# the-lay/voltools

Hardware: AMD Instinct MI355X
Metric: Mvoxels/s, 512^3 f32 filt_bspline StaticVolume transform (resident source, device output) (higher is better)
Workload: dtype f32; 1 GPU; 512^3 float32 filt_bspline, StaticVolume resident in HBM, rotate((0,i,0)) rzxz sweep, output= device buffer; lds_bytes=34816, kernel=8, resident_bytes=1660944384, angles=i

## Files before the change

include/voltools_hip.h:

```cpp
#ifndef VOLTOOLS_HIP_H
#define VOLTOOLS_HIP_H

#include <stddef.h>
#include <stdint.h>

#ifdef __cplusplus
extern "C" {
#endif

enum vt_interp {
    VT_LINEAR = 0,
    VT_BSPLINE = 1,
    VT_BSPLINE_SIMPLE = 2,
    VT_FILT_BSPLINE = 3,
    VT_FILT_BSPLINE_SIMPLE = 4
};

enum vt_flags {
    VT_OUT_DEVICE = 1,
    VT_KEEP_OUTSIDE = 2,
    VT_FORCE_DIRECT = 4,
    VT_FORCE_TILED = 8,
    VT_NO_ZSEP = 16,
    VT_NO_MARCH = 32,
    VT_NO_ZPAIR = 64,
    VT_NO_PACKED = 128,
    VT_FORCE_PACKED = 256,
    VT_FORCE_XSWAP = 512,
    VT_NO_RSWAP = 1024,
    VT_ONESHOT_EDGE_SCIPY = 4096,
    VT_NO_QUAD = 2048,
    VT_NO_BLOCK = 8192,
    VT_NO_ZFIR = 16384,
    VT_NO_REORIENT = 32768,
    VT_NO_ROWS = 65536,
    VT_NO_PLANSHARE = 131072
};

enum vt_create_flags {
    VT_SRC_DEVICE = 1,
    VT_SLAB_LO_INTERIOR = 2,
    VT_SLAB_HI_INTERIOR = 4,
    VT_EDGE_SCIPY = 16,
    VT_SRC_DEFERRED = 8
};

enum vt_error {
    VT_OK = 0,
    VT_EINVAL = 10001,
    VT_ENODEV = 10002,
    VT_ENOMEM = 10003,
    VT_EUNSUPPORTED = 10004
};

typedef struct vt_volume vt_volume_t;

typedef struct vt_volume_info {
    int32_t device;
    int32_t interp;
    int32_t depth, height, width;
    int32_t out_depth, out_height, out_width;
    int32_t last_kernel;
    int32_t last_tile[3];
    int32_t last_lds_dims[3];
    int32_t last_lds_bytes;
    int32_t last_grid;
    float   prefilter_ms;
    uint64_t resident_bytes;
    float   copies_ms;
    int32_t copies_built;
    int32_t copies_evicted;
    uint64_t max_resident_bytes;
} vt_volume_info_t;

int vt_device_count(int* count);
int vt_device_name(int dev, char* buf, int buflen);
int vt_device_props(int dev, int* cu_count, int* lds_bytes_per_block, uint64_t* hbm_bytes);
int vt_device_synchronize(int dev);

int vt_malloc(int dev, size_t bytes, void** dptr);
int vt_free(int dev, void* dptr);
int vt_memset_zero(int dev, void* dptr, size_t bytes);
int vt_memcpy_h2d(int dev, void* dptr, const void* hptr, size_t bytes);
int vt_memcpy_d2h(int dev, void* hptr, const void* dptr, size_t bytes);
int vt_memcpy_d2d(int dev, void* dst, const void* src, size_t bytes);
int vt_host_register(int dev, void* ptr, size_t bytes);
int vt_host_unregister(int dev, void* ptr);
int vt_device_trim(int dev);

// ... 73 lines not shown
```

voltools_amd/_native.py:

```python
import ctypes
import os
from typing import Optional, Tuple

import numpy as np

_HERE = os.path.dirname(os.path.abspath(__file__))
LIB_PATH = os.environ.get('VT_LIB') or os.path.join(_HERE, 'lib', 'libvoltools_hip.so')

INTERP_CODES = {'linear': 0, 'bspline': 1, 'bspline_simple': 2, 'filt_bspline': 3, 'filt_bspline_simple': 4}

OUT_DEVICE, KEEP_OUTSIDE, FORCE_DIRECT, FORCE_TILED, NO_ZSEP, NO_MARCH, NO_ZPAIR, NO_PACKED, FORCE_PACKED, FORCE_XSWAP, NO_RSWAP, NO_QUAD, ONESHOT_EDGE_SCIPY, NO_BLOCK, NO_ZFIR, NO_REORIENT, NO_ROWS, NO_PLANSHARE = 1, 2, 4, 8, 16, 32, 64, 128, 256, 512, 1024, 2048, 4096, 8192, 16384, 32768, 65536, 131072
SRC_DEVICE, SLAB_LO_INTERIOR, SLAB_HI_INTERIOR, SRC_DEFERRED, EDGE_SCIPY = 1, 2, 4, 8, 16

SYMBOLS = [
    'vt_device_count', 'vt_device_name', 'vt_device_props', 'vt_device_synchronize',
    'vt_malloc', 'vt_free', 'vt_memset_zero', 'vt_memcpy_h2d', 'vt_memcpy_d2h', 'vt_memcpy_d2d',
    'vt_host_register', 'vt_host_unregister', 'vt_device_trim',
    'vt_volume_create', 'vt_volume_create_slab', 'vt_volume_upload_planes', 'vt_volume_finalize', 'vt_volume_destroy', 'vt_volume_info', 'vt_volume_stream',
    'vt_volume_sync', 'vt_volume_set_output_shape', 'vt_volume_affine', 'vt_volume_affine_f64',
    'vt_volume_project', 'vt_volume_project_f64', 'vt_volume_affine_batch',
    'vt_timer_start', 'vt_timer_stop', 'vt_prefilter_inplace', 'vt_affine_oneshot',
    'vt_last_error', 'vt_version', 'vt_has_legacy_kernels', 'vt_volume_release_copies', 'vt_volume_set_max_resident',
    'vt_volume_extract', 'vt_volume_extract_f64', 'vt_volume_project_batch', 'vt_volume_project_batch_f64',
    'vt_volume_extract_sum', 'vt_volume_extract_sum_f64', 'vt_volume_extract_dot', 'vt_volume_extract_dot_f64',
    'vt_volume_extract_dot_multi', 'vt_volume_extract_dot_multi_f64',
]


class VolumeInfo(ctypes.Structure):
    _fields_ = [('device', ctypes.c_int32), ('interp', ctypes.c_int32),
                ('depth', ctypes.c_int32), ('height', ctypes.c_int32), ('width', ctypes.c_int32),
                ('out_depth', ctypes.c_int32), ('out_height', ctypes.c_int32), ('out_width', ctypes.c_int32),
                ('last_kernel', ctypes.c_int32), ('last_tile', ctypes.c_int32 * 3),
                ('last_lds_dims', ctypes.c_int32 * 3), ('last_lds_bytes', ctypes.c_int32),
                ('last_grid', ctypes.c_int32), ('prefilter_ms', ctypes.c_float),
                ('resident_bytes', ctypes.c_uint64), ('copies_ms', ctypes.c_float), ('copies_built', ctypes.c_int32),
                ('copies_evicted', ctypes.c_int32), ('max_resident_bytes', ctypes.c_uint64)]


_lib = None


def _preload_hip_runtime():
    import importlib.util
    import sys
    if os.environ.get('VT_HIP_RUNTIME', '') == 'system' or 'torch' in sys.modules:
        return
    try:
        spec = importlib.util.find_spec('torch')
    except (ImportError, ValueError):
        spec = None
    if spec is None or not spec.submodule_search_locations:
        return
    cand = os.path.join(list(spec.submodule_search_locations)[0], 'lib', 'libamdhip64.so')
    if os.path.exists(cand):
        try:
            ctypes.CDLL(cand, mode=ctypes.RTLD_GLOBAL)
        except OSError:
            pass


def load():
    global _lib
    if _lib is not None:
# ... 278 lines not shown
```

voltools_amd/csrc/vt_kernels_quad.hip:

```cpp
#include "vt_internal.h"
#include <cstdio>
#include <cstdlib>
#include <mutex>
#include <unordered_map>
#include "vt_device.h"
#include "vt_march_common.h"

#include <type_traits>

namespace vt {

typedef float v4f __attribute__((ext_vector_type(4)));

constexpr int kQuadMaxIt = 5;

template <int NT> constexpr int quad_plan_granules() { return (kTabInts + NT * kQuadMaxIt / 4 + 2) / 3; }
constexpr int quad_plan_vote_off(int granules) { return kTabBytes + ((12 * granules + 15) & ~15); }
constexpr int quad_plan_lds_bytes(int granules, int nt) { return quad_plan_vote_off(granules) + 4 * (nt / 64); }

__global__ __launch_bounds__(256) void relayout_zquad(const float* __restrict__ src, float* __restrict__ dst,
                                                       int D, int H, int W, int P, int Pq)
{
    const int x = blockIdx.x * 256 + threadIdx.x;
    const int y = blockIdx.y;
// ... 150 lines not shown
                    const float x0 = fmaf(fx, a01 - a00, a00);
                    const float x1 = fmaf(fx, a11 - a10, a10);
                    pl[c] = fmaf(fy, x1 - x0, x0);
                }
                val = fmaf(p.fz, pl[1] - pl[0], pl[0]);
            } else if constexpr (KIND == 4) {
                const int z = d + p.zoff;
                float accy = 0.f;
#pragma unroll
                for (int bb = 0; bb < 4; ++bb) {
                    const int y = gy0 - 1 + bb;
                    float accx = wx[0] * fetch(z, y, gx0 - 1);
                    accx = fmaf(wx[1], fetch(z, y, gx0), accx);
                    accx = fmaf(wx[2], fetch(z, y, gx0 + 1), accx);
                    accx = fmaf(wx[3], fetch(z, y, gx0 + 2), accx);
                    accy = fmaf(wy[bb], accx, accy);
                }
                val = accy;
            } else {
#pragma unroll
                for (int c = 0; c < 4; ++c) {
                    const int z = d + p.zoff - 1 + c;
                    float accy = 0.f;
#pragma unroll
                    for (int bb = 0; bb < 4; ++bb) {
                        const int y = gy0 - 1 + bb;
                        float accx = wx[0] * fetch(z, y, gx0 - 1);
                        accx = fmaf(wx[1], fetch(z, y, gx0), accx);
                        accx = fmaf(wx[2], fetch(z, y, gx0 + 1), accx);
                        accx = fmaf(wx[3], fetch(z, y, gx0 + 2), accx);
                        accy = fmaf(wy[bb], accx, accy);
                    }
                    val = (c == 0) ? wz[0] * accy : fmaf(wz[c], accy, val);
                }
            }
            out[oo + (int64_t)d * p.ostride] = val;
        } else if (!keep) out[oo + (int64_t)d * p.ostride] = 0.0f;
    }
}

__device__ __forceinline__ int quad_lane_to_pos(int lane)
{
    const int blk = (lane >> 2) & 7;
    const int sh = (int)((0x30051663u >> (4 * blk)) & 15u) - 3;
    return lane + 4 * sh;
}
__device__ __forceinline__ int quad_pos_to_lane(int pos)
{
    const int blk = (pos >> 2) & 7;
    const int sh = (int)((0x31006653u >> (4 * blk)) & 15u) - 3;
    return pos + 4 * sh;
}

template <int KIND, int TH, int TW, int NT>
__global__ __launch_bounds__(NT, (KIND == 4 && TH * TW == 2 * NT) ? 4 : 1) void affine_march4(const float* __restrict__ srcq, float* __restrict__ out, const AffineParams p)
{
    static_assert(NT % TW == 0 && TH % (NT / TW) == 0 && NT % 64 == 0 && 64 % TW == 0, "tile/thread mapping");
    static_assert(NT == 256 || NT == 512, "quad_tile_plan_granules");
    static_assert(quad_plan_granules<NT>() <= NT && 3 * quad_plan_granules<NT>() <= kTabInts + kVrowCap / 4, "one plan granule per thread");
    constexpr bool CUBIC = KIND == 1 || KIND == 2 || KIND == 4;
    constexpr bool ZID = KIND == 3 || KIND == 4;
    constexpr int HALO = CUBIC ? 1 : 0;
    constexpr int ZH = ZID ? 0 : HALO;
    constexpr int NR = 2 + 2 * HALO;
    constexpr int NC = 2 * ZH + 1;
    constexpr int ZNEW = ZID ? 0 : 1;
    constexpr int RP = NT / TW;
    constexpr int NPIX = TH / RP;
    constexpr int NSTORE = 4 * NPIX;
    extern __shared__ __attribute__((aligned(16))) float lds[];

    const int tid = threadIdx.x;
#ifdef VT_EXPERIMENTS
    if ((p.flags & (1 << 27)) && (p.flags & (1 << 26))) return;
    long long stamp[5];
    stamp[0] = clock64();
#endif
    int tw_i, th_i, chunk;
    if (p.flags & (1 << 29)) {
        chunk = (p.flags & (1 << 20)) ? (int)(gridDim.y - 1 - blockIdx.y) : (int)blockIdx.y;
        unsigned u = (unsigned)xcd_contiguous(blockIdx.x, gridDim.x);
        if (p.flags & (1 << 30)) u = gridDim.x - 1 - u;
        if (p.flags & (1 << 24)) {
            tw_i = (int)__umulhi(u, p.nTh_magic);
            th_i = (int)u - tw_i * p.nTh;
        } else {
            th_i = (int)__umulhi(u, p.nTw_magic);
            tw_i = (int)u - th_i * p.nTw;
        }
    } else {
        int t = xcd_contiguous(blockIdx.x, gridDim.x);
        if (p.flags & (1 << 20)) t = (int)gridDim.x - 1 - t;
        march_tile(p, t, th_i, tw_i, chunk);
    }
    const int h0 = th_i * TH, w0 = tw_i * TW;
    constexpr int PG = quad_plan_granules<NT>();
    const bool share = KIND == 4 && p.tplan != nullptr;
    int4 pgran = {0, 0, 0, 0};
    int4* const plan_g = share ? reinterpret_cast<int4*>(p.tplan) + (int64_t)(th_i * p.nTw + tw_i) * PG : nullptr;
    if (share && tid < PG) {
        const __amdgpu_buffer_rsrc_t prsrc = __builtin_amdgcn_make_buffer_rsrc(plan_g, 0, PG * 16, 0x00020000);
        pgran = __builtin_bit_cast(int4, __builtin_amdgcn_raw_buffer_load_b128(prsrc, 16 * tid, 0, 16));
    }
    const int d_begin = chunk ? chunk * p.dch + p.dshift : 0;
    const int d_end = min((chunk + 1) * p.dch + p.dshift, p.oD);

    double base[3], lo[3], hi[3];
    bool any_valid = true, all_valid = true;
#pragma unroll
    for (int r = 1; r < 3; ++r) {
        base[r] = fma(p.m[4 * r + 1], (double)h0, fma(p.m[4 * r + 2], (double)w0, p.m[4 * r + 3]));
        lo[r] = base[r] + p.neg[r];
        hi[r] = base[r] + p.pos[r];
        any_valid = any_valid && (hi[r] >= p.vlo[r] - kTileMargin) && (lo[r] < p.vhi[r] + kTileMargin);
        all_valid = all_valid && (lo[r] >= p.vlo[r] + kTileMargin) && (hi[r] < p.vhi[r] - kTileMargin);
    }
    const double z_lo = (double)d_begin + p.m[3], z_hi = (double)(d_end - 1) + p.m[3];
    any_valid = any_valid && (z_hi >= p.vlo[0] - kTileMargin) && (z_lo < p.vhi[0] + kTileMargin);
    all_valid = all_valid && (z_lo >= p.vlo[0] + kTileMargin) && (z_hi < p.vhi[0] - kTileMargin);
    const bool keep = (p.flags & VT_KEEP_OUTSIDE) != 0;
    const int64_t ostride = p.ostride, orow = p.orow;
    const bool lane_perm = (p.flags & (1 << 23)) != 0;
    const int lane_id = tid & 63;
    const int pos = lane_perm ? quad_lane_to_pos(lane_id) : lane_id;
    const int kw = pos % TW;
    const int jh0 = (tid >> 6) * (64 / TW) + pos / TW;
    const int lane_left = lane_perm ? quad_pos_to_lane((pos + 63) & 63) : ((lane_id + 63) & 63);
    const int lane_right = lane_perm ? quad_pos_to_lane((pos + 1) & 63) : ((lane_id + 1) & 63);

    if (!any_valid) {
        if (!keep) {
#pragma unroll
            for (int px = 0; px < NPIX; ++px) {
                const int h = h0 + jh0 + px * RP, w = w0 + kw;
                if (h < p.oH && w < p.oW) {
                    float* optr = out + (int64_t)d_begin * ostride + (int64_t)h * orow + w;
                    for (int d = d_begin; d < d_end; ++d, optr += ostride) *optr = 0.0f;
                }
            }
        }
        return;
    }

    int o1, o2;
    {
        const int f1 = (int)floor(lo[1]), f2 = (int)floor(lo[2]);
        int g1 = f1, g2 = f2;
        asm volatile("" : "+v"(g1), "+v"(g2));
        o1 = __builtin_amdgcn_readfirstlane(g1);
        o2 = __builtin_amdgcn_readfirstlane(g2);
        o1 -= HALO;
        o2 -= HALO;
    }

    int iy[NPIX], ix[NPIX];
    float fy[NPIX], fx[NPIX];
    float wy[NPIX][4], wx[NPIX][4];
    bool in_yx[NPIX], pix_ok[NPIX];
    int ob[NPIX];
    const double by = base[1] - (double)o1, bx = base[2] - (double)o2;
#pragma unroll
    for (int px = 0; px < NPIX; ++px) {
        const int j = jh0 + px * RP;
        const double sy = fma(p.m[5], (double)j, fma(p.m[6], (double)kw, by));
        const double sx = fma(p.m[9], (double)j, fma(p.m[10], (double)kw, bx));
        const double fyd = floor(sy), fxd = floor(sx);
        fy[px] = (float)(sy - fyd);
        fx[px] = (float)(sx - fxd);
        iy[px] = (int)fyd;
        ix[px] = (int)fxd;
        if constexpr (KIND == 4) {
            if (p.flags & (1 << 18)) { cubic_weights<true>(fy[px], wy[px]); cubic_weights<true>(fx[px], wx[px]); }
            else { cubic_weights<false>(fy[px], wy[px]); cubic_weights<false>(fx[px], wx[px]); }
        } else if constexpr (CUBIC) { cubic_weights<KIND == 2>(fy[px], wy[px]); cubic_weights<KIND == 2>(fx[px], wx[px]); }
        else {
#pragma unroll
            for (int k = 0; k < 4; ++k) { wy[px][k] = 0.f; wx[px][k] = 0.f; }
        }
        in_yx[px] = all_valid || (canonical_inside_axis(p, 1, 0, h0 + j, w0 + kw) && canonical_inside_axis(p, 2, 0, h0 + j, w0 + kw));
        pix_ok[px] = (h0 + j < p.oH) && (w0 + kw < p.oW);
        ob[px] = (int)(((int64_t)j * orow + kw) * 4);
    }

#ifdef VT_EXPERIMENTS
    stamp[1] = clock64();
#endif
    int voff[kQuadMaxIt];
    int q[NPIX][NR];
    int nvec;
    {
        int* tab = reinterpret_cast<int*>(lds);
#ifdef VT_QUAD_ANALYTIC_SPANS
        build_span_table<TH, TW, HALO, 1>(tab, p, p.Ly, by, bx, tid);
#else
        if (tid < 2 * kRowsMax) tab[tid] = (tid < kRowsMax) ? 0x7fffffff : (int)0x80000000;
        int* const img = reinterpret_cast<int*>(reinterpret_cast<char*>(lds) + kTabBytes);
        int* const vote = reinterpret_cast<int*>(reinterpret_cast<char*>(lds) + quad_plan_vote_off(PG));
        if (share) {
            if (tid < PG) { img[3 * tid] = pgran.x; img[3 * tid + 1] = pgran.y; img[3 * tid + 2] = pgran.z; }
            const bool wave_ok = __all(tid >= PG || (unsigned)pgran.w == p.tplan_epoch);
            if ((tid & 63) == 0) vote[tid >> 6] = wave_ok ? 1 : 0;
        }
        __syncthreads();
        bool hit = false;
        if (share) {
            int all = 1;
#pragma unroll
            for (int w = 0; w < NT / 64; ++w) all &= vote[w];
            hit = __builtin_amdgcn_readfirstlane(all) != 0;
        }
        if (hit) {
            tab = img;
#ifdef VT_EXPERIMENTS
            stamp[2] = stamp[3] = clock64();
#endif
        } else {
            unsigned char* vrow = reinterpret_cast<unsigned char*>(tab + kTabInts);
#pragma unroll
            for (int px = 0; px < NPIX; ++px) {
                const int iy_l = __shfl(iy[px], lane_left), iy_r = __shfl(iy[px], lane_right);
                const bool edge = (kw == 0) || (kw == TW - 1) || (iy_l != iy[px]) || (iy_r != iy[px]);
                if (edge) {
#pragma unroll
                    for (int r = 0; r < NR; ++r) {
                        const int row = min(max(iy[px] - HALO + r, 0), kRowsMax - 1);
                        atomicMin(&tab[row], ix[px] - HALO);
                        atomicMax(&tab[kRowsMax + row], ix[px] + HALO + 1);
                    }
                }
            }
            __syncthreads();
#ifdef VT_EXPERIMENTS
            stamp[2] = clock64();
#endif
            if (tid < kRowsMax) {
                const int lane = tid;
                const int mn = tab[lane], mx = tab[kRowsMax + lane];
                const bool used = mn <= mx;
                const int x0 = used ? mn : 0;
                const int nv = used ? (mx - mn + 1) : 0;
                int first, pad = 0, total;
                {
                    const int incl = wave_scan_add(nv);
                    first = incl - nv;
                    total = __builtin_amdgcn_readlane(incl, 63);
                }
                if (p.row_s >= 0) {
                    const int S = p.row_s;
                    const int c_r = (x0 + lane * S) & 15;
                    const int end_res = (nv > 0) ? ((c_r + nv) & 15) : 0;
                    const int last_used = wave_scan_max((nv > 0) ? lane : -1);
                    const int prev_row = wave_shift_up1(last_used, -1);
                    int prev_end = __shfl(end_res, max(prev_row, 0));
                    if (lane == 0 || prev_row < 0) prev_end = 0;
                    const int gap = (nv > 0) ? ((c_r - prev_end) & 15) : 0;
                    const int inc2 = wave_scan_add(gap + nv);
// ... 9 lines not shown
                int v = first;
                for (; v < last && (v & 3); ++v) vrow[v] = (unsigned char)lane;
                const unsigned lane4 = (unsigned)lane * 0x01010101u;
                for (; v + 4 <= last; v += 4) *reinterpret_cast<unsigned*>(vrow + v) = lane4;
                for (; v < last; ++v) vrow[v] = (unsigned char)lane;
            }
            __syncthreads();
#ifdef VT_EXPERIMENTS
            stamp[3] = clock64();
#endif
            if (share && tid < PG) {
                const int nvb = min(tab[2 * kRowsMax], NT * kQuadMaxIt);
                int w[3];
#pragma unroll
                for (int j = 0; j < 3; ++j) {
                    const int k = 3 * tid + j;
                    const int b = 4 * (k - kTabInts);
                    int val = 0;
                    if (k <= 2 * kRowsMax) val = tab[k];
                    else if (k >= kTabInts && b < nvb) val = tab[k] & ((b + 4 <= nvb) ? -1 : (int)((1u << (8 * (nvb - b))) - 1u));
                    w[j] = val;
                }
                plan_g[tid] = make_int4(w[0], w[1], w[2], (int)p.tplan_epoch);
            }
        }
#endif
        const unsigned char* vrow = reinterpret_cast<const unsigned char*>(tab + kTabInts);
        nvec = tab[2 * kRowsMax];
#pragma unroll
        for (int it = 0; it < kQuadMaxIt; ++it) {
            const int v = tid + NT * it;
            const int y = (v < nvec && v < kVrowCap) ? vrow[v] : 255;
            const int yy = (y == 255) ? 0 : y;
            const int cx = v - tab[kRowsMax + yy];
            const int gy = o1 + yy, gx = o2 + tab[yy] + cx;
            const bool ok = (y != 255) && (unsigned)gy < (unsigned)p.sH && (unsigned)gx < (unsigned)p.sW;
            voff[it] = ok ? (gy * p.sPq + 4 * gx) * 4 : p.zero_off_q;
        }
#pragma unroll
        for (int px = 0; px < NPIX; ++px) {
#pragma unroll
            for (int r = 0; r < NR; ++r) {
                const int row = min(max(iy[px] - HALO + r, 0), kRowsMax - 1);
                q[px][r] = 16 * (tab[kRowsMax + row] + (ix[px] - HALO - tab[row]));
            }
        }
        __syncthreads();
    }
#pragma unroll
    for (int it = 0; it < kQuadMaxIt; ++it) voff[it] -= p.zero_off_q;
    const int nvec64 = (nvec + 63) & ~63;
    const int slot_bytes = p.slot_floats * 4;

    if (nvec64 * 16 > slot_bytes || nvec64 > NT * kQuadMaxIt) {
#pragma unroll
        for (int px = 0; px < NPIX; ++px)
            if (pix_ok[px])
                quad_gather_column<KIND>(srcq, out, p, (int64_t)(h0 + jh0 + px * RP) * orow + (w0 + kw), d_begin, d_end, in_yx[px],
                                         o1 + iy[px], o2 + ix[px], fy[px], fx[px]);
        return;
    }

    const int wave_first = __builtin_amdgcn_readfirstlane(tid & ~63);
    const int quad_bytes = p.sH * p.sPq * 4;
    const int nquads_res = (p.sD + 3) >> 2;
    const int plane_first = d_begin + p.zoff - ZH, plane_last = d_end - 1 + p.zoff + ZH + ZNEW;
    const int Q0 = floordiv4(plane_first), QN = floordiv4(plane_last);
    const int Q_base = max(0, min(Q0, nquads_res - 1));
    __amdgpu_buffer_rsrc_t rsrc = __builtin_amdgcn_make_buffer_rsrc(
        const_cast<char*>(reinterpret_cast<const char*>(srcq) + (int64_t)Q_base * quad_bytes), 0, 0x7fffffff, 0x00020000);
    __amdgpu_buffer_rsrc_t orsrc = __builtin_amdgcn_make_buffer_rsrc(
        reinterpret_cast<char*>(out + ((int64_t)d_begin * ostride + (int64_t)h0 * orow + w0)), 0, 0x7fffffff, 0x00020000);
    const int oplane_bytes = (int)(ostride * 4);
    const float fz = p.fz;
    float wz[4] = {0.f, 0.f, 0.f, 0.f};
    if constexpr (CUBIC && !ZID) cubic_weights<KIND == 2>(fz, wz);
    const int tap_new = p.zoff + ZH + ZNEW;
    const int Qf0 = floordiv4(d_begin + tap_new + 3), Qf1 = floordiv4(d_end - 4 + tap_new);
    const bool nt_stores = (p.flags & (1 << 28)) != 0;
    const bool tile_fast = all_valid && (h0 + TH <= p.oH) && (w0 + TW <= p.oW);
    char* const lds_c = reinterpret_cast<char*>(lds);
#ifdef VT_EXPERIMENTS
    const bool no_stores = (p.flags & (1 << 21)) != 0, no_loads = (p.flags & (1 << 22)) != 0, no_lds = (p.flags & (1 << 26)) != 0;
#else
    constexpr bool no_stores = false, no_loads = false, no_lds = false;
#endif
#ifdef VT_EXPERIMENTS
    if (p.flags & (1 << 27)) {
        if (nvec == 12345678) out[0] = (float)(voff[0] + q[0][0]);
        stamp[4] = clock64();
        if (tid == 0) {
            const int64_t b = (int64_t)blockIdx.x + (int64_t)gridDim.x * blockIdx.y;
            for (int k = 0; k < 4; ++k) out[b * 4 + k] = (float)(stamp[k + 1] - stamp[k]);
        }
        return;
    }
#endif

    auto run = [&](auto nit_c) {
        constexpr int NIT = decltype(nit_c)::value;
        const bool last_wave = wave_first + NT * (NIT - 1) < nvec64;
        auto issue_quad = [&](int Q, int slot_off) {
            if (no_loads) return;
            const bool quad_ok = (unsigned)Q < (unsigned)nquads_res;
            const int soff = quad_ok ? (Q - Q_base) * quad_bytes : 0;
            const int okmask = quad_ok ? -1 : 0;
            char* dst = lds_c + slot_off + 16 * wave_first;
#pragma unroll
            for (int it = 0; it < NIT; ++it) {
                const int off = p.zero_off_q + (voff[it] & okmask);
                if (it + 1 < NIT || last_wave)
                    __builtin_amdgcn_raw_ptr_buffer_load_lds(rsrc, (__attribute__((address_space(3))) void*)(dst + (16 * NT) * it), 16, off, soff, 0, 0);
            }
        };

        float carry[NPIX][NC];
#pragma unroll
        for (int px = 0; px < NPIX; ++px)
#pragma unroll
            for (int c = 0; c < NC; ++c) carry[px][c] = 0.f;

        auto partials = [&](int slot_off, v4f (&part)[NPIX]) {
            if (no_lds) {
#pragma unroll
                for (int px = 0; px < NPIX; ++px) asm volatile("" : "=v"(part[px]));
                return;
            }
            const char* sl = lds_c + slot_off;
#pragma unroll
            for (int px = 0; px < NPIX; ++px) {
                if constexpr (!CUBIC) {
                    const v4f a00 = *reinterpret_cast<const v4f*>(sl + q[px][0]);
                    const v4f a01 = *reinterpret_cast<const v4f*>(sl + q[px][0] + 16);
                    const v4f a10 = *reinterpret_cast<const v4f*>(sl + q[px][1]);
                    const v4f a11 = *reinterpret_cast<const v4f*>(sl + q[px][1] + 16);
                    const v4f x0 = (a01 - a00) * fx[px] + a00;
                    const v4f x1 = (a11 - a10) * fx[px] + a10;
                    part[px] = (x1 - x0) * fy[px] + x0;
                } else {
                    v4f accy = {0.f, 0.f, 0.f, 0.f};
#pragma unroll
                    for (int bb = 0; bb < 4; ++bb) {
                        const char* rowp = sl + q[px][bb];
                        const v4f t0 = *reinterpret_cast<const v4f*>(rowp);
                        const v4f t1 = *reinterpret_cast<const v4f*>(rowp + 16);
                        const v4f t2 = *reinterpret_cast<const v4f*>(rowp + 32);
                        const v4f t3 = *reinterpret_cast<const v4f*>(rowp + 48);
                        v4f accx = t0 * wx[px][0];
                        accx = t1 * wx[px][1] + accx;
                        accx = t2 * wx[px][2] + accx;
                        accx = t3 * wx[px][3] + accx;
                        accy = accx * wy[px][bb] + accy;
                    }
                    part[px] = accy;
                }
            }
        };
        auto zcombine = [&](int px, float pn) -> float {
            float val;
            if constexpr (ZID) {
                val = pn;
            } else if constexpr (!CUBIC) {
                val = fmaf(fz, pn - carry[px][0], carry[px][0]);
                carry[px][0] = pn;
            } else {
                float acc = wz[0] * carry[px][0];
                acc = fmaf(wz[1], carry[px][1], acc);
                acc = fmaf(wz[2], carry[px][2], acc);
                val = fmaf(wz[3], pn, acc);
                carry[px][0] = carry[px][1]; carry[px][1] = carry[px][2]; carry[px][2] = pn;
            }
            return val;
        };

        int slot_off = 0;
        issue_quad(Q0, 0);
        bool prev_full = false;
        for (int Q = Q0; Q <= QN; ++Q) {
            const bool full = tile_fast && Q >= Qf0 && Q <= Qf1;
            if (full && prev_full && !no_stores) asm volatile("s_waitcnt vmcnt(%0)" ::"n"(NSTORE) : "memory");
            else asm volatile("s_waitcnt vmcnt(0)" ::: "memory");
            __builtin_amdgcn_s_barrier();
            if (Q < QN) issue_quad(Q + 1, slot_off ^ slot_bytes);
            v4f part[NPIX];
            partials(slot_off, part);
            const int d_first = 4 * Q - tap_new;
            if (full) {
                int soff = (d_first - d_begin) * oplane_bytes;
                float val[4][NPIX];
#pragma unroll
                for (int i = 0; i < 4; ++i)
#pragma unroll
                    for (int px = 0; px < NPIX; ++px) val[i][px] = zcombine(px, part[px][i]);
                if (no_stores) {
#pragma unroll
                    for (int i = 0; i < 4; ++i)
#pragma unroll
                        for (int px = 0; px < NPIX; ++px) asm volatile("" ::"v"(val[i][px]));
                } else if (nt_stores) {
#pragma unroll
                    for (int i = 0; i < 4; ++i, soff += oplane_bytes)
#pragma unroll
                        for (int px = 0; px < NPIX; ++px)
                            __builtin_amdgcn_raw_buffer_store_b32(__builtin_bit_cast(unsigned, val[i][px]), orsrc, ob[px], soff, 2);
                } else {
#pragma unroll
                    for (int i = 0; i < 4; ++i, soff += oplane_bytes)
#pragma unroll
                        for (int px = 0; px < NPIX; ++px)
                            __builtin_amdgcn_raw_buffer_store_b32(__builtin_bit_cast(unsigned, val[i][px]), orsrc, ob[px], soff, 0);
                }
            } else {
#pragma unroll
                for (int i = 0; i < 4; ++i) {
                    const int d = d_first + i;
                    const bool d_ok = (d >= d_begin) && (d < d_end);
                    const double ez = (double)d + p.m[3];
                    const bool z_ok = (ez >= p.vlo[0]) && (ez < p.vhi[0]);
                    const int soff = (d - d_begin) * oplane_bytes;
#pragma unroll
                    for (int px = 0; px < NPIX; ++px) {
                        const float val = zcombine(px, part[px][i]);
                        if (d_ok && pix_ok[px]) {
                            if (in_yx[px] && z_ok) __builtin_amdgcn_raw_buffer_store_b32(__builtin_bit_cast(unsigned, val), orsrc, ob[px], soff, 0);
                            else if (!keep) __builtin_amdgcn_raw_buffer_store_b32(0u, orsrc, ob[px], soff, 0);
                        }
                    }
                }
            }
            prev_full = full;
            slot_off ^= slot_bytes;
        }
    };
    using std::integral_constant;
    switch (nvec64 / NT + ((nvec64 % NT) ? 1 : 0)) {
        case 1: run(integral_constant<int, 1>{}); break;
        case 2: run(integral_constant<int, 2>{}); break;
        case 3: run(integral_constant<int, 3>{}); break;
        case 4: run(integral_constant<int, 4>{}); break;
        default: run(integral_constant<int, 5>{}); break;
    }
}

typedef void (*quad_fn)(const float*, float*, const AffineParams);
struct QuadCfg { int th, tw, nt; };
static const QuadCfg kQuad[] = {
    {16, 32, 256},
    {8, 32, 256},
    {32, 32, 256},
    {16, 64, 256},
    {32, 32, 512},
    {16, 64, 512},
};
int quad_max_it() { return kQuadMaxIt; }
int quad_config_count() { return (int)(sizeof(kQuad) / sizeof(kQuad[0])); }
void quad_config(int idx, int* th, int* tw, int* nt) { *th = kQuad[idx].th; *tw = kQuad[idx].tw; *nt = kQuad[idx].nt; }
int quad_tile_plan_granules(int cfg) { return kQuad[cfg].nt == 512 ? quad_plan_granules<512>() : quad_plan_granules<256>(); }
int quad_tile_plan_lds(int cfg) { return quad_plan_lds_bytes(quad_tile_plan_granules(cfg), kQuad[cfg].nt); }

template <int TH, int TW, int NT>
static quad_fn pick_quad(int kind)
{
    switch (kind) {
        case 0: return affine_march4<0, TH, TW, NT>;
        case 1: return affine_march4<1, TH, TW, NT>;
        case 3: return affine_march4<3, TH, TW, NT>;
        case 4: return affine_march4<4, TH, TW, NT>;
        default: return affine_march4<2, TH, TW, NT>;
    }
}
static quad_fn quad_entry(int cfg, int kind)
{
    switch (cfg) {
        case 0: return pick_quad<16, 32, 256>(kind);
        case 1: return pick_quad<8, 32, 256>(kind);
        case 2: return pick_quad<32, 32, 256>(kind);
        case 3: return pick_quad<16, 64, 256>(kind);
        case 4: return pick_quad<32, 32, 512>(kind);
        default: return pick_quad<16, 64, 512>(kind);
    }
}

hipError_t init_quad_kernels()
{
    for (int cfg = 0; cfg < quad_config_count(); ++cfg)
        for (int kind = 0; kind < 5; ++kind) {
            hipError_t e = hipFuncSetAttribute(reinterpret_cast<const void*>(quad_entry(cfg, kind)),
                                               hipFuncAttributeMaxDynamicSharedMemorySize, 160 * 1024);
            if (e != hipSuccess) return e;
        }
    return hipSuccess;
}

int quad_blocks_per_cu(int cfg, int interp, int lds_bytes, bool zid)
// ... 34 lines not shown
```

voltools_amd/csrc/vt_plan.hip:

```cpp
#include "vt_host.h"
#include "vt_device.h"

#include <cmath>
#include <cstring>

namespace vt {
namespace {

struct PlanCtx {
    const vt_volume* v;
    const double* m;
    int flags;
    AffineParams* p;
    TilePlan* plan;
    bool cubic;
    bool zsep;
    int halo2;
};

#ifdef VT_LEGACY
int64_t round_aware_chunks(int64_t oD, int g, int64_t inplane, int64_t resident, int64_t n0, int extra, int min_dch, int64_t n_floor)
{
    if (resident <= 0 || inplane > resident || inplane * n0 >= 16 * resident) return n0;
    auto cost = [&](int64_t n) {
// ... 230 lines not shown
                p->row_s = S;
                nvec64 = padded64;
            }
        }
        const int slot_bytes = nvec64 * 16;
        const int64_t bytes = std::max<int64_t>(2LL * slot_bytes, march_table_bytes());
        if (bytes > v->lds_limit) continue;
        c.plan->kind = 8; c.plan->cfg = cfg; c.plan->td = 4; c.plan->th = th; c.plan->tw = tw;
        c.plan->lds_bytes = (int)bytes;
        p->Lz = 2; p->Ly = std::min(L[1], march_rows_max()); p->Lx = npos; p->Lx_used = npos;
        p->slot_floats = slot_bytes / 4;
        return true;
    }
    return false;
}

bool plan_quad(PlanCtx& c)
{
    const vt_volume* v = c.v;
    AffineParams* p = c.p;
    TilePlan* plan = c.plan;
    if (!c.zsep || (c.flags & (VT_NO_MARCH | VT_NO_QUAD | VT_NO_ZPAIR))) return false;
    if (v->H > 65535 || (v->D + 3) / 4 > 65535) return false;
    const bool zfir = c.cubic && (float)(c.m[3] - std::floor(c.m[3])) == 0.0f && v->tune.quad_zfir != 0 && !(c.flags & VT_NO_ZFIR);
    const int halo = (c.cubic && !zfir) ? 1 : 0;
    const int Wq = (v->W + 1 + 7) & ~7;
    const int64_t quad_bytes = (int64_t)v->H * Wq * 16;
    if (quad_bytes >= 0x7fffffffLL) return false;
    const int64_t max_stride = (int64_t)std::max(v->oD, v->oH) * v->oW;
    const TilePlan saved = *plan;
    if (!quad_pick_tile(c, max_stride)) return false;
    const int T[3] = {1, plan->th, plan->tw};
    set_tile_reach(p, c.m, T, 1);
    set_axis0_split(p, c.m);
    p->nTh = (v->oH + plan->th - 1) / plan->th;
    p->nTw = (v->oW + plan->tw - 1) / plan->tw;
    p->sPq = 4 * Wq;
    p->zero_off_q = v->W * 16;
    p->flags = (c.flags & VT_KEEP_OUTSIDE) | experiment_flags(v);
    if (v->tune.quad_nt < 0 ? true : v->tune.quad_nt != 0) p->flags |= (1 << 28);
    if (v->tune.quad_perm != 0) p->flags |= (1 << 23);
    const bool zid = !c.cubic && p->fz == 0.0f && v->tune.quad_zid != 0;
    if (zid) p->flags |= (1 << 25);
    if (zfir && p->fz == 0.0f) {
        p->flags |= (1 << 19);
        if (v->interp == VT_BSPLINE_SIMPLE || v->interp == VT_FILT_BSPLINE_SIMPLE) p->flags |= (1 << 18);
    }
    const bool zfir_on = (p->flags & (1 << 19)) != 0;
    const bool share_plans = zfir_on && !(c.flags & VT_NO_PLANSHARE);
    if (share_plans) {
        p->flags |= (1 << 17);
        plan->lds_bytes = std::max(plan->lds_bytes, quad_tile_plan_lds(plan->cfg));
    }
    const bool one_plane = zid || zfir_on;
    const int64_t inplane = (int64_t)p->nTh * p->nTw;
    int target_dch = c.cubic ? 64 : (((int64_t)v->H * v->W <= 512 * 512) ? 24 : 32);
    if (zfir_on) target_dch = share_plans ? 24 : 32;
    if (zid) target_dch = 16;
    if (one_plane && v->tune.zid_dch > 0) target_dch = v->tune.zid_dch;
    if (v->tune.dch > 0) target_dch = std::max(4, v->tune.dch);
    int64_t nchunks = std::max<int64_t>(1, (v->oD + target_dch - 1) / target_dch);
    if (v->tune.dch <= 0)
        nchunks = std::max(nchunks, std::min<int64_t>((4 * (int64_t)v->cu_count + inplane - 1) / inplane, (v->oD + 7) / 8));
    const int64_t n_addr = std::max(((int64_t)(v->oD / 4 + 4) * quad_bytes) / 0x60000000LL + 1, ((int64_t)v->oD * max_stride * 4) / 0x60000000LL + 1);
    nchunks = std::max<int64_t>(nchunks, n_addr);
    plan->blocks_per_cu = quad_blocks_per_cu(plan->cfg, v->interp, plan->lds_bytes, one_plane);
    int dch = (int)((v->oD + nchunks - 1) / nchunks);
    dch = (dch + 3) & ~3;
    const int dshift = (int)((((int64_t)halo - (int64_t)p->zoff) % 4 + 4) % 4);
    nchunks = (v->oD > dshift) ? (v->oD - dshift + dch - 1) / dch : 1;
    const int64_t grid = inplane * nchunks;
    if ((int64_t)(dch + dshift) * max_stride * 4 >= 0x7fffffffLL || grid > 0x7fffffffLL) { *plan = saved; return false; }
    p->dch = dch;
    p->dshift = dshift;
    p->nTd = (int)nchunks;
    if (v->tune.blk_h > 0 && v->tune.blk_w > 0) { p->blk_h = v->tune.blk_h; p->blk_w = v->tune.blk_w; }
    plan->grid = (int)grid;
    const bool grid2d = (v->tune.quad_grid2d != 0) && p->blk_h <= 0 && nchunks <= 65535 && inplane * std::max(p->nTh, p->nTw) < (1LL << 32) &&
                        p->nTw > 1 && p->nTh > 1;
    if (grid2d) {
        p->nTw_magic = (uint32_t)((1ULL << 32) / (uint64_t)p->nTw + 1);
        p->nTh_magic = (uint32_t)((1ULL << 32) / (uint64_t)p->nTh + 1);
        p->flags |= (1 << 29);
        const bool rev = v->tune.quad_reverse >= 0 ? v->tune.quad_reverse != 0 : c.m[5] < 0.0;
        if (rev) p->flags |= (1 << 30);
    }
    return true;
}

#ifdef VT_LEGACY
bool zpair_pick_tile(PlanCtx& c)
{
    const vt_volume* v = c.v;
    AffineParams* p = c.p;
    const double* m = c.m;
    for (int cfg = 0; cfg < zpair_config_count(); ++cfg) {
        if (v->tune.tile >= 0 && cfg != v->tune.tile) continue;
        int th, tw, la, nt;
        zpair_config(cfg, &th, &tw, &la, &nt);
        if (v->tune.la > 0) la = std::min(3, v->tune.la);
        const int vec_max = nt * march_max_it();
        int L[3];
        if (!inplane_box(m, th, tw, c.halo2, L)) continue;
        L[2] = (L[2] + 1 + 1) & ~1;
        bool zp_box = true;
        if (v->tune.march_box >= 0) zp_box = v->tune.march_box != 0;
// ... 639 lines not shown
```

Measured before the change: 703,600 Mvoxels/s.

## Share cubic B-spline taps between vertically paired output pixels in quad march kernel

Adds a tap-sharing mode for the two-pixel-per-thread cubic quad kernel. When the paired pixels map to adjacent source rows, the second pixel reuses the first pixel's LDS row loads, and its weights are permuted so the overlapping rows and columns are computed once. The weighted sums use packed f32 multiply and FMA instructions through inline asm. Neighbouring rows are assigned to the same thread, with a per-workgroup vote that falls back to direct gathering if any wave's offsets don't qualify. This is meant to cut LDS reads and VALU work per voxel, at the cost of more template instantiations, extra register pressure and added setup logic.

New measurement: 700,600 Mvoxels/s. Within noise of the previous version (-0.4%).

```diff
diff --git a/include/voltools_hip.h b/include/voltools_hip.h
--- a/include/voltools_hip.h
+++ b/include/voltools_hip.h
@@ -34,7 +34,8 @@
     VT_NO_ZFIR = 16384,
     VT_NO_REORIENT = 32768,
     VT_NO_ROWS = 65536,
-    VT_NO_PLANSHARE = 131072
+    VT_NO_PLANSHARE = 131072,
+    VT_NO_TAPSHARE = 262144
 };
 
 enum vt_create_flags {
diff --git a/voltools_amd/_native.py b/voltools_amd/_native.py
--- a/voltools_amd/_native.py
+++ b/voltools_amd/_native.py
@@ -9,7 +9,7 @@
 
 INTERP_CODES = {'linear': 0, 'bspline': 1, 'bspline_simple': 2, 'filt_bspline': 3, 'filt_bspline_simple': 4}
 
-OUT_DEVICE, KEEP_OUTSIDE, FORCE_DIRECT, FORCE_TILED, NO_ZSEP, NO_MARCH, NO_ZPAIR, NO_PACKED, FORCE_PACKED, FORCE_XSWAP, NO_RSWAP, NO_QUAD, ONESHOT_EDGE_SCIPY, NO_BLOCK, NO_ZFIR, NO_REORIENT, NO_ROWS, NO_PLANSHARE = 1, 2, 4, 8, 16, 32, 64, 128, 256, 512, 1024, 2048, 4096, 8192, 16384, 32768, 65536, 131072
+OUT_DEVICE, KEEP_OUTSIDE, FORCE_DIRECT, FORCE_TILED, NO_ZSEP, NO_MARCH, NO_ZPAIR, NO_PACKED, FORCE_PACKED, FORCE_XSWAP, NO_RSWAP, NO_QUAD, ONESHOT_EDGE_SCIPY, NO_BLOCK, NO_ZFIR, NO_REORIENT, NO_ROWS, NO_PLANSHARE, NO_TAPSHARE = 1, 2, 4, 8, 16, 32, 64, 128, 256, 512, 1024, 2048, 4096, 8192, 16384, 32768, 65536, 131072, 262144
 SRC_DEVICE, SLAB_LO_INTERIOR, SLAB_HI_INTERIOR, SRC_DEFERRED, EDGE_SCIPY = 1, 2, 4, 8, 16
 
 SYMBOLS = [
diff --git a/voltools_amd/csrc/vt_kernels_quad.hip b/voltools_amd/csrc/vt_kernels_quad.hip
--- a/voltools_amd/csrc/vt_kernels_quad.hip
+++ b/voltools_amd/csrc/vt_kernels_quad.hip
@@ -226,6 +226,46 @@
     return pos + 4 * sh;
 }
 
+typedef float v2f __attribute__((ext_vector_type(2)));
+template <int H> __device__ __forceinline__ v2f pk_mul_b(v2f t, v2f w)
+{
+    v2f r;
+    if constexpr (H == 0) asm("v_pk_mul_f32 %0, %1, %2 op_sel_hi:[1,0]" : "=v"(r) : "v"(t), "v"(w));
+    else asm("v_pk_mul_f32 %0, %1, %2 op_sel:[0,1] op_sel_hi:[1,1]" : "=v"(r) : "v"(t), "v"(w));
+    return r;
+}
+template <int H> __device__ __forceinline__ v2f pk_fma_b(v2f t, v2f w, v2f c)
+{
+    v2f r;
+    if constexpr (H == 0) asm("v_pk_fma_f32 %0, %1, %2, %3 op_sel_hi:[1,0,1]" : "=v"(r) : "v"(t), "v"(w), "v"(c));
+    else asm("v_pk_fma_f32 %0, %1, %2, %3 op_sel:[0,1,0] op_sel_hi:[1,1,1]" : "=v"(r) : "v"(t), "v"(w), "v"(c));
+    return r;
+}
+template <int H> __device__ __forceinline__ v2f pk_fma_b0(v2f t, v2f w)
+{
+    v2f r;
+    if constexpr (H == 0) asm("v_pk_fma_f32 %0, %1, %2, 0 op_sel_hi:[1,0,0]" : "=v"(r) : "v"(t), "v"(w));
+    else asm("v_pk_fma_f32 %0, %1, %2, 0 op_sel:[0,1,0] op_sel_hi:[1,1,0]" : "=v"(r) : "v"(t), "v"(w));
+    return r;
+}
+template <int H> __device__ __forceinline__ v4f mul_b(v4f t, v2f w)
+{
+    const v2f lo = pk_mul_b<H>(t.lo, w), hi = pk_mul_b<H>(t.hi, w);
+    return v4f{lo.x, lo.y, hi.x, hi.y};
+}
+template <int H> __device__ __forceinline__ v4f fma_b(v4f t, v2f w, v4f c)
+{
+    const v2f lo = pk_fma_b<H>(t.lo, w, c.lo), hi = pk_fma_b<H>(t.hi, w, c.hi);
+    return v4f{lo.x, lo.y, hi.x, hi.y};
+}
+template <int H> __device__ __forceinline__ v4f fma_b0(v4f t, v2f w)
+{
+    const v2f lo = pk_fma_b0<H>(t.lo, w), hi = pk_fma_b0<H>(t.hi, w);
+    return v4f{lo.x, lo.y, hi.x, hi.y};
+}
+
+template <class T> __device__ __forceinline__ T pick(bool c, T a, T b) { return c ? a : b; }
+
 template <int KIND, int TH, int TW, int NT>
 __global__ __launch_bounds__(NT, (KIND == 4 && TH * TW == 2 * NT) ? 4 : 1) void affine_march4(const float* __restrict__ srcq, float* __restrict__ out, const AffineParams p)
 {
@@ -299,6 +339,10 @@
     const int pos = lane_perm ? quad_lane_to_pos(lane_id) : lane_id;
     const int kw = pos % TW;
     const int jh0 = (tid >> 6) * (64 / TW) + pos / TW;
+    constexpr bool PAIR = KIND == 4 && NPIX == 2;
+    const bool tapshare = PAIR && (p.flags & (1 << 15)) != 0;
+    const int pair_sw = (tapshare && p.m[5] < 0.0) ? 1 : 0;
+    auto pix_row = [&](int px) -> int { return tapshare ? 2 * jh0 + (px ^ pair_sw) : jh0 + px * RP; };
     const int lane_left = lane_perm ? quad_pos_to_lane((pos + 63) & 63) : ((lane_id + 63) & 63);
     const int lane_right = lane_perm ? quad_pos_to_lane((pos + 1) & 63) : ((lane_id + 1) & 63);
 
@@ -306,7 +350,7 @@
         if (!keep) {
 #pragma unroll
             for (int px = 0; px < NPIX; ++px) {
-                const int h = h0 + jh0 + px * RP, w = w0 + kw;
+                const int h = h0 + pix_row(px), w = w0 + kw;
                 if (h < p.oH && w < p.oW) {
                     float* optr = out + (int64_t)d_begin * ostride + (int64_t)h * orow + w;
                     for (int d = d_begin; d < d_end; ++d, optr += ostride) *optr = 0.0f;
@@ -335,7 +379,7 @@
     const double by = base[1] - (double)o1, bx = base[2] - (double)o2;
 #pragma unroll
     for (int px = 0; px < NPIX; ++px) {
-        const int j = jh0 + px * RP;
+        const int j = pix_row(px);
         const double sy = fma(p.m[5], (double)j, fma(p.m[6], (double)kw, by));
         const double sx = fma(p.m[9], (double)j, fma(p.m[10], (double)kw, bx));
         const double fyd = floor(sy), fxd = floor(sx);
@@ -356,6 +400,18 @@
         ob[px] = (int)(((int64_t)j * orow + kw) * 4);
     }
 
+    int ts_mode = 0;
+    bool ts_dy1 = false, ts_sh = false;
+    if constexpr (PAIR) {
+        if (tapshare) {
+            const bool xneg = (pair_sw ? -p.m[9] : p.m[9]) < 0.0;
+            const int dx = ix[1] - ix[0], dy = iy[1] - iy[0];
+            if (__all((unsigned)dy <= 1u && (unsigned)(xneg ? -dx : dx) <= 1u)) ts_mode = __all(dx == 0) ? 2 : (xneg ? 3 : 1);
+            ts_dy1 = dy != 0;
+            ts_sh = xneg ? (dx != 0) : (dx == 0);
+        }
+    }
+    bool ts_fail = false;
 #ifdef VT_EXPERIMENTS
     stamp[1] = clock64();
 #endif
@@ -368,6 +424,9 @@
         build_span_table<TH, TW, HALO, 1>(tab, p, p.Ly, by, bx, tid);
 #else
         if (tid < 2 * kRowsMax) tab[tid] = (tid < kRowsMax) ? 0x7fffffff : (int)0x80000000;
+        unsigned char* const ts_vote = reinterpret_cast<unsigned char*>(tab + 2 * kRowsMax + 1);
+        static_assert(NT / 64 <= 4 * (kTabInts - 2 * kRowsMax - 1), "one vote byte per wave");
+        if (tapshare && (tid & 63) == 0) ts_vote[tid >> 6] = ts_mode != 0 ? 1 : 0;
         int* const img = reinterpret_cast<int*>(reinterpret_cast<char*>(lds) + kTabBytes);
         int* const vote = reinterpret_cast<int*>(reinterpret_cast<char*>(lds) + quad_plan_vote_off(PG));
         if (share) {
@@ -376,6 +435,12 @@
             if ((tid & 63) == 0) vote[tid >> 6] = wave_ok ? 1 : 0;
         }
         __syncthreads();
+        if (tapshare) {
+            int all = 1;
+#pragma unroll
+            for (int w = 0; w < NT / 64; ++w) all &= ts_vote[w];
+            ts_fail = __builtin_amdgcn_readfirstlane(all) == 0;
+        }
         bool hit = false;
         if (share) {
             int all = 1;
@@ -491,11 +556,11 @@
     const int nvec64 = (nvec + 63) & ~63;
     const int slot_bytes = p.slot_floats * 4;
 
-    if (nvec64 * 16 > slot_bytes || nvec64 > NT * kQuadMaxIt) {
+    if (nvec64 * 16 > slot_bytes || nvec64 > NT * kQuadMaxIt || ts_fail) {
 #pragma unroll
         for (int px = 0; px < NPIX; ++px)
             if (pix_ok[px])
-                quad_gather_column<KIND>(srcq, out, p, (int64_t)(h0 + jh0 + px * RP) * orow + (w0 + kw), d_begin, d_end, in_yx[px],
+                quad_gather_column<KIND>(srcq, out, p, (int64_t)(h0 + pix_row(px)) * orow + (w0 + kw), d_begin, d_end, in_yx[px],
                                          o1 + iy[px], o2 + ix[px], fy[px], fx[px]);
         return;
     }
@@ -536,8 +601,33 @@
     }
 #endif
 
-    auto run = [&](auto nit_c) {
+    if constexpr (PAIR) {
+        if (ts_mode != 0) {
+            float vy[4], vx[4];
+#pragma unroll
+            for (int k = 0; k < 4; ++k) {
+                vy[k] = wy[1][k];
+                vx[k] = wx[1][k];
+                asm("" : "+v"(vy[k]), "+v"(vx[k]));
+            }
+            const int own1 = pick(ts_dy1, q[1][3], q[1][0]);
+            const float e = pick(ts_dy1, vy[3], vy[0]);
+            const float m0 = pick(ts_dy1, vy[0], vy[1]), m1 = pick(ts_dy1, vy[1], vy[2]), m2 = pick(ts_dy1, vy[2], vy[3]);
+            wy[1][0] = e; wy[1][1] = m0; wy[1][2] = m1; wy[1][3] = m2;
+            q[1][0] = own1;
+            if (ts_mode != 2) {
+                q[1][0] = own1 + (ts_sh ? 16 : 0);
+                q[1][1] = ts_sh ? -16 : 48;
+                const float xe = pick(ts_sh, vx[0], vx[3]);
+                const float x0 = pick(ts_sh, vx[1], vx[0]), x1 = pick(ts_sh, vx[2], vx[1]), x2 = pick(ts_sh, vx[3], vx[2]);
+                wx[1][0] = xe; wx[1][1] = x0; wx[1][2] = x1; wx[1][3] = x2;
+            }
+        }
+    }
+
+    auto run = [&](auto nit_c, auto ts_c) {
         constexpr int NIT = decltype(nit_c)::value;
+        constexpr int TS = decltype(ts_c)::value;
         const bool last_wave = wave_first + NT * (NIT - 1) < nvec64;
         auto issue_quad = [&](int Q, int slot_off) {
             if (no_loads) return;
@@ -559,6 +649,24 @@
 #pragma unroll
             for (int c = 0; c < NC; ++c) carry[px][c] = 0.f;
 
+        v2f X0a = {0.f, 0.f}, X0b = X0a, Y0a = X0a, Y0b = X0a, X1e = X0a, X1m = X0a, X1f = X0a, Y1e = X0a, Y1m = X0a, XY2 = X0a;
+        if constexpr (TS != 0) {
+            X0a = v2f{wx[0][0], wx[0][1]}; X0b = v2f{wx[0][2], wx[0][3]};
+            Y0a = v2f{wy[0][0], wy[0][1]}; Y0b = v2f{wy[0][2], wy[0][3]};
+            Y1e = v2f{ts_dy1 ? 0.f : wy[1][0], ts_dy1 ? wy[1][0] : 0.f};
+            Y1m = v2f{wy[1][1], wy[1][2]};
+            if constexpr (TS == 2) {
+                X1e = v2f{wx[1][0], wx[1][1]};
+                X1m = v2f{wx[1][2], wx[1][3]};
+                XY2 = v2f{0.f, wy[1][3]};
+            } else {
+                X1e = v2f{ts_sh ? 0.f : wx[1][2], wx[1][1]};
+                X1m = v2f{ts_sh ? wx[1][0] : 0.f, ts_sh ? wx[1][2] : 0.f};
+                X1f = v2f{wx[1][3], ts_sh ? 0.f : wx[1][0]};
+                XY2 = v2f{0.f, wy[1][3]};
+            }
+        }
+
         auto partials = [&](int slot_off, v4f (&part)[NPIX]) {
             if (no_lds) {
 #pragma unroll
@@ -566,6 +674,72 @@
                 return;
             }
             const char* sl = lds_c + slot_off;
+            if constexpr (TS != 0) {
+                static_assert(NPIX == 2 && CUBIC, "tap sharing: cubic vertical pairs");
+                auto ld = [&](const char* ptr) -> v4f { return *reinterpret_cast<const v4f*>(ptr); };
+                v4f acc0, acc1, own1;
+                {
+                    const char* rowp = sl + q[0][0];
+                    const v4f t0 = ld(rowp), t1 = ld(rowp + 16), t2 = ld(rowp + 32), t3 = ld(rowp + 48);
+                    v4f accx;
+                    accx = mul_b<1>(t1, X0a);
+                    accx = fma_b<0>(t0, X0a, accx);
+                    accx = fma_b<0>(t2, X0b, accx);
+                    accx = fma_b<1>(t3, X0b, accx);
+                    acc0 = fma_b0<0>(accx, Y0a);
+                }
+                {
+                    const char* rowp = sl + q[1][0];
+                    const v4f u0 = ld(rowp), u1 = ld(rowp + 16), u2 = ld(rowp + 32);
+                    if constexpr (TS == 2) {
+                        const v4f u3 = ld(rowp + 48);
+                        own1 = mul_b<1>(u1, X1e);
+                        own1 = fma_b<0>(u0, X1e, own1);
+                        own1 = fma_b<0>(u2, X1m, own1);
+                        own1 = fma_b<1>(u3, X1m, own1);
+                    } else {
+                        const v4f ue = ld(rowp + q[1][1]);
+                        own1 = fma_b0<0>(u1, X1e);
+                        own1 = fma_b<1>(u0, X1e, own1);
+                        own1 = fma_b<0>(ue, X1m, own1);
+                        own1 = fma_b<1>(u1, X1m, own1);
+                        own1 = fma_b<0>(u2, X1f, own1);
+                        own1 = fma_b<1>(ue, X1f, own1);
+                    }
+                    acc1 = fma_b0<0>(own1, Y1e);
+                }
+#pragma unroll
+                for (int i = 0; i < 3; ++i) {
+                    const char* rowp = sl + q[0][i + 1];
+                    const v4f t0 = ld(rowp), t1 = ld(rowp + 16), t2 = ld(rowp + 32), t3 = ld(rowp + 48);
+                    v4f x0;
+                    x0 = mul_b<1>(t1, X0a);
+                    x0 = fma_b<0>(t0, X0a, x0);
+                    x0 = fma_b<0>(t2, X0b, x0);
+                    x0 = fma_b<1>(t3, X0b, x0);
+                    acc0 = (i == 0) ? fma_b<1>(x0, Y0a, acc0) : (i == 1) ? fma_b<0>(x0, Y0b, acc0) : fma_b<1>(x0, Y0b, acc0);
+                    v4f x1;
+                    if constexpr (TS == 2) {
+                        x1 = mul_b<1>(t1, X1e);
+                        x1 = fma_b<0>(t0, X1e, x1);
+                        x1 = fma_b<0>(t2, X1m, x1);
+                        x1 = fma_b<1>(t3, X1m, x1);
+                    } else {
+                        const v4f te = ld(rowp + q[1][1] + (TS == 1 ? 16 : 0));
+                        const v4f s0 = (TS == 1) ? t1 : t0, s1 = (TS == 1) ? t2 : t1, s2 = (TS == 1) ? t3 : t2;
+                        x1 = fma_b0<0>(s1, X1e);
+                        x1 = fma_b<1>(s0, X1e, x1);
+                        x1 = fma_b<0>(te, X1m, x1);
+                        x1 = fma_b<1>(s1, X1m, x1);
+                        x1 = fma_b<0>(s2, X1f, x1);
+                        x1 = fma_b<1>(te, X1f, x1);
+                    }
+                    acc1 = (i == 0) ? fma_b<0>(x1, Y1m, acc1) : (i == 1) ? fma_b<1>(x1, Y1m, acc1) : fma_b<1>(x1, XY2, acc1);
+                }
+                part[0] = acc0;
+                part[1] = fma_b<1>(own1, Y1e, acc1);
+                return;
+            }
 #pragma unroll
             for (int px = 0; px < NPIX; ++px) {
                 if constexpr (!CUBIC) {
@@ -672,13 +846,22 @@
         }
     };
     using std::integral_constant;
-    switch (nvec64 / NT + ((nvec64 % NT) ? 1 : 0)) {
-        case 1: run(integral_constant<int, 1>{}); break;
-        case 2: run(integral_constant<int, 2>{}); break;
-        case 3: run(integral_constant<int, 3>{}); break;
-        case 4: run(integral_constant<int, 4>{}); break;
-        default: run(integral_constant<int, 5>{}); break;
-    }
+    const int nit_wg = __builtin_amdgcn_readfirstlane(nvec64 / NT + ((nvec64 % NT) ? 1 : 0));
+    auto run_nit = [&](auto ts_c) {
+        switch (nit_wg) {
+            case 1: run(integral_constant<int, 1>{}, ts_c); break;
+            case 2: run(integral_constant<int, 2>{}, ts_c); break;
+            case 3: run(integral_constant<int, 3>{}, ts_c); break;
+            case 4: run(integral_constant<int, 4>{}, ts_c); break;
+            default: run(integral_constant<int, 5>{}, ts_c); break;
+        }
+    };
+    if constexpr (PAIR) {
+        if (ts_mode == 0) { run_nit(integral_constant<int, 0>{}); return; }
+        if (ts_mode == 1) { run_nit(integral_constant<int, 1>{}); return; }
+        if (ts_mode == 2) { run_nit(integral_constant<int, 2>{}); return; }
+        run_nit(integral_constant<int, 3>{});
+    } else run_nit(integral_constant<int, 0>{});
 }
 
 typedef void (*quad_fn)(const float*, float*, const AffineParams);
diff --git a/voltools_amd/csrc/vt_plan.hip b/voltools_amd/csrc/vt_plan.hip
--- a/voltools_amd/csrc/vt_plan.hip
+++ b/voltools_amd/csrc/vt_plan.hip
@@ -306,6 +306,12 @@
         p->flags |= (1 << 17);
         plan->lds_bytes = std::max(plan->lds_bytes, quad_tile_plan_lds(plan->cfg));
     }
+    {
+        int th, tw, nt;
+        quad_config(plan->cfg, &th, &tw, &nt);
+        if (zfir_on && !(c.flags & VT_NO_TAPSHARE) && th * tw == 2 * nt && std::fabs(c.m[5]) <= 1.0 && std::fabs(c.m[9]) <= 1.0)
+            p->flags |= (1 << 15);
+    }
     const bool one_plane = zid || zfir_on;
     const int64_t inplane = (int64_t)p->nTh * p->nTw;
     int target_dch = c.cubic ? 64 : (((int64_t)v->H * v->W <= 512 * 512) ? 24 : 32);
```
